# huzjkevin/planar_optical_flow

Hardware: AMD Instinct MI355X
Metric: scans/sec, flow-only preprocess of 450-pt synthetic scan pairs, batch 4096 per GPU (+ flow EPE vs reference oracle) (higher is better)
Workload: dtype f32 flow arithmetic (float32 outputs) + f64 exact association / mask decisions; the float64-output instantiation (the reference's float64 operation order) is `value_f64`

## Files before the change

### planar_optical_flow_amd/csrc/scan_flow.hip

```cpp
#include <cmath>
#include <type_traits>

#include "pof_common.h"

namespace {

constexpr int kThreads = 256;
constexpr int kFlatThreads = 128;
constexpr int kFlatRuns = 1;
constexpr int kFlatPairs = 64 * kFlatRuns;

__global__ void laser_phi_kernel(double start, double stop, double step, int n, double *tab)
{
    int i = blockIdx.x * blockDim.x + threadIdx.x;
    if (i >= n) return;
    double p = (double)i * step;
    p = p + start;
    if (i == n - 1 && n > 1) p = stop;
    double s, c;
    sincos(p, &s, &c);
    tab[i] = p;
    tab[n + 2 * i] = c;
    tab[n + 2 * i + 1] = s;
}
// ... 269 lines not shown
    if (a->det_offsets && slot >= cnt) {
        reinterpret_cast<float4 *>(img + kImgScreen)[slot] = make_float4(0.0f, 0.0f, INFINITY, 0.0f);
        img[40 + slot] = 0;
    }
}

__global__ __launch_bounds__(256) void scan_params_kernel(PreArgs a)
{
    params_work<true, true>(&a, blockIdx.x * blockDim.x + threadIdx.x);
}

__device__ __forceinline__ double to_sgpr(double v)
{
    const int lo = __builtin_amdgcn_readfirstlane(__double2loint(v));
    const int hi = __builtin_amdgcn_readfirstlane(__double2hiint(v));
    return __hiloint2double(hi, lo);
}

#define GLOBAL_AS __attribute__((address_space(1)))
using F4V = float __attribute__((ext_vector_type(4)));
using F2V = float __attribute__((ext_vector_type(2)));
using LL2V = long long __attribute__((ext_vector_type(2)));
__device__ __forceinline__ void stream_f4(float *base, long long idx4, float x, float y, float z, float w)
{
    F4V v = {x, y, z, w};
    __builtin_nontemporal_store(v, (GLOBAL_AS F4V *)base + idx4);
}
__device__ __forceinline__ void stream_f2(float *base, long long idx2, float x, float y)
{
    F2V v = {x, y};
    __builtin_nontemporal_store(v, (GLOBAL_AS F2V *)base + idx2);
}
__device__ __forceinline__ void stream_ll2(long long *base, long long idx2, long long x, long long y)
{
    LL2V v = {x, y};
    __builtin_nontemporal_store(v, (GLOBAL_AS LL2V *)base + idx2);
}

template <typename OutT>
__device__ __forceinline__ void store2(OutT *base, long long idx, double a, double b)
{
    using V = OutT __attribute__((ext_vector_type(2)));
    V v = {(OutT)a, (OutT)b};
    ((GLOBAL_AS V *)base)[idx] = v;
}

constexpr int kDetTile = 32;

__device__ __forceinline__ float4 prefilter_entry(double cx, double cy, double sd, double sa)
{
    const bool far = !(fabs(cx) + fabs(cy) < 100.0);
    return make_float4((float)cx, (float)cy, (float)sd, far ? INFINITY : (float)sa);
}

template <typename OutT, int PTS, int SPB>
__device__ __forceinline__ void scan_main(const PreArgs &a, const int block_y)
{
    __shared__ double s_det[SPB][kDetTile][5];
    __shared__ int s_lab[SPB][kDetTile];
    __shared__ float4 s_detf[SPB][kDetTile];

    const int b0 = block_y * SPB;
    const int tid = threadIdx.x;
    const int i0 = (blockIdx.x * kThreads + tid) * PTS;
    const int N = a.N;
    const bool live = i0 < N;
    const bool want_flow = a.flow != nullptr;
    const bool want_assoc = a.det_offsets != nullptr;

    int ndet[SPB];
    float r[SPB][PTS];
    double mot[SPB][7];
#pragma unroll
    for (int q = 0; q < SPB; ++q) {
        const int b = min(b0 + q, a.B - 1);
        const float *row = a.ranges + (long long)b * a.sample_stride;
#pragma unroll
        for (int k = 0; k < PTS; ++k) r[q][k] = 0.0f;
        if (live) {
            if (PTS == 2) {
                float2 v = *reinterpret_cast<const float2 *>(row + i0);
                r[q][0] = v.x;
                r[q][PTS - 1] = v.y;
            } else {
                r[q][0] = row[i0];
            }
        }
#pragma unroll
        for (int c = 0; c < 7; ++c) mot[q][c] = 0.0;
        ndet[q] = 0;
        if (want_flow || want_assoc) {
            typedef const __attribute__((address_space(4))) double *cptr;
            cptr m = (cptr)(a.ws_rec + (long long)b * kRecStride);
#pragma unroll
            for (int c = 0; c < 7; ++c) mot[q][c] = m[c];
            ndet[q] = (int)m[7];
        }
    }
    double cs[PTS], sn[PTS];
#pragma unroll
    for (int k = 0; k < PTS; ++k) cs[k] = sn[k] = 0.0;
    if (live) {
#pragma unroll
        for (int k = 0; k < PTS; ++k) {
            double2 t = *reinterpret_cast<const double2 *>(a.tab + N + 2 * (i0 + k));
            cs[k] = t.x;
            sn[k] = t.y;
        }
    }
    if (want_assoc) {
        const int qsel = tid / kInline, j = tid - qsel * kInline;
#pragma unroll
        for (int q = 0; q < SPB; ++q) {
            if (qsel == q) {
                const int b = min(b0 + q, a.B - 1);
                const double *w = a.ws_rec + (long long)b * kRecStride + 8 + j * kDetStride;
                s_det[q][j][0] = w[0];
                s_det[q][j][1] = w[1];
                s_det[q][j][2] = w[2];
                s_det[q][j][3] = w[3];
                s_det[q][j][4] = w[5];
                s_lab[q][j] = (int)w[4];
                s_detf[q][j] = prefilter_entry(w[0], w[1], w[3], w[5]);
            }
        }
    }
    bool synced = false;

#pragma unroll
    for (int q = 0; q < SPB; ++q) {
        const int b = b0 + q;
        const bool ok = live && b < a.B;
        double px[PTS], py[PTS];
#pragma unroll
        for (int k = 0; k < PTS; ++k) {
            px[k] = (double)r[q][k] * cs[k];
            py[k] = (double)r[q][k] * sn[k];
        }
        float pxf[PTS], pyf[PTS];
        bool far[PTS];
#pragma unroll
        for (int k = 0; k < PTS; ++k) {
            pxf[k] = (float)px[k];
            pyf[k] = (float)py[k];
            far[k] = !(fabsf(pxf[k]) + fabsf(pyf[k]) < 100.0f);
        }
        const long long o = (long long)b * N + i0;

        if (ok && a.xy) {
            OutT *xy = static_cast<OutT *>(a.xy);
#pragma unroll
            for (int k = 0; k < PTS; ++k) store2<OutT>(xy, o + k, px[k], py[k]);
        }

        if (ok && want_flow) {
            OutT *fl = static_cast<OutT *>(a.flow);
            const double m0 = mot[q][0], m1 = mot[q][1], m2 = mot[q][2], m3 = mot[q][3];
            const double t0 = mot[q][4], t1 = mot[q][5], dph = mot[q][6];
            double fxs[PTS], fys[PTS];
#pragma unroll
            for (int k = 0; k < PTS; ++k) {
                double fx, fy;
                apply_motion(a.flow_kind, px[k], py[k], m0, m1, m2, m3, t0, t1, dph, fx, fy);
                if (a.canonical) {
                    double gx = cs[k] * fx + (-sn[k]) * fy;
                    double gy = sn[k] * fx + cs[k] * fy;
                    fx = gx;
                    fy = gy;
                }
                fxs[k] = fx;
                fys[k] = fy;
            }
            if (PTS == 2 && sizeof(OutT) == 4) {
                stream_f4(reinterpret_cast<float *>(fl), o / 2, (float)fxs[0], (float)fys[0], (float)fxs[PTS - 1],
                          (float)fys[PTS - 1]);
            } else {
#pragma unroll
                for (int k = 0; k < PTS; ++k) store2<OutT>(fl, o + k, fxs[k], fys[k]);
            }
        }

        float vmask[PTS], dmask[PTS];
#pragma unroll
        for (int k = 0; k < PTS; ++k) {
            vmask[k] = (r[q][k] >= 20.0f) ? 0.0f : 1.0f;
            dmask[k] = 1.0f;
        }

        if (want_assoc) {
            double best[PTS];
            int bidx[PTS];
#pragma unroll
            for (int k = 0; k < PTS; ++k) {
                best[k] = 0.0;
                bidx[k] = 0;
            }
            if (!synced) {
                __syncthreads();
                synced = true;
            }
            int dfirst = 0;
            if (ndet[q] > kInline) dfirst = a.det_offsets[min(b, a.B - 1)];
            for (int base = 0; base < ndet[q]; base += (base == 0 ? kInline : kDetTile)) {
                const int cnt = min(base == 0 ? kInline : kDetTile, ndet[q] - base);
                if (base != 0) {
                    __syncthreads();
                    if (tid < cnt) {
                        const double *w = a.ws_det + (long long)(dfirst + base + tid) * kDetStride;
                        s_det[q][tid][0] = w[0];
                        s_det[q][tid][1] = w[1];
                        s_det[q][tid][2] = w[2];
                        s_det[q][tid][3] = w[3];
                        s_det[q][tid][4] = w[5];
                        s_lab[q][tid] = (int)w[4];
                        s_detf[q][tid] = prefilter_entry(w[0], w[1], w[3], w[5]);
                    }
                    __syncthreads();
                }
                float4 fnext = s_detf[q][0];
                for (int j = 0; j < cnt; ++j) {
                    const float4 f = fnext;
                    fnext = s_detf[q][min(j + 1, kDetTile - 1)];
                    bool exact[PTS];
                    bool any_exact = false;
#pragma unroll
                    for (int k = 0; k < PTS; ++k) {
                        const float exf = pxf[k] - f.x, eyf = pyf[k] - f.y;
                        const float s2f = fmaf(exf, exf, eyf * eyf);
                        const float mgn = fmaf(s2f, 1e-4f, 1e-3f);
                        exact[k] = far[k] || (s2f - mgn < f.w) || (fabsf(s2f - f.z) <= mgn);
                        if (!exact[k] && s2f < f.z) dmask[k] = 0.0f;
                        any_exact |= exact[k];
                    }
                    if (any_exact) {
                        const double cx = s_det[q][j][0], cy = s_det[q][j][1];
                        const double sd = s_det[q][j][3], sa = s_det[q][j][4];
#pragma unroll
                        for (int k = 0; k < PTS; ++k) {
                            if (!exact[k]) continue;
                            const double ex = px[k] - cx, ey = py[k] - cy;
                            const double s2 = ex * ex + ey * ey;
                            if (s2 <= sd) dmask[k] = 0.0f;
                            if (s2 <= sa) {
                                const double v = sqrt(s2) - s_det[q][j][2];
                                if (v < best[k]) {
                                    best[k] = v;
                                    bidx[k] = base + j + 1;
                                }
                            }
                        }
                    }
                }
            }
            if (ok) {
                long long cls[PTS];
                float gx[PTS], gy[PTS];
#pragma unroll
                for (int k = 0; k < PTS; ++k) {
                    cls[k] = 0;
                    gx[k] = gy[k] = 0.0f;
                    if (bidx[k] > 0) {
                        double wx, wy;
                        if (ndet[q] <= kInline) {
                            wx = s_det[q][bidx[k] - 1][0];
                            wy = s_det[q][bidx[k] - 1][1];
                            cls[k] = s_lab[q][bidx[k] - 1];
                        } else {
                            const double *w = a.ws_det + (long long)(dfirst + bidx[k] - 1) * kDetStride;
                            wx = w[0];
                            wy = w[1];
                            cls[k] = (long long)w[4];
                        }
                        gx[k] = (float)(wy * cs[k] - wx * sn[k]);
                        gy[k] = (float)((wx * cs[k] + wy * sn[k]) - (double)r[q][k]);
                    }
                }
                if (PTS == 2) {
                    if (a.closest) stream_ll2(reinterpret_cast<long long *>(a.closest), o / 2, bidx[0], bidx[PTS - 1]);
                    if (a.target_cls) stream_ll2(reinterpret_cast<long long *>(a.target_cls), o / 2, cls[0], cls[PTS - 1]);
                    if (a.target_reg) stream_f4(a.target_reg, o / 2, gx[0], gy[0], gx[PTS - 1], gy[PTS - 1]);
                } else {
                    if (a.closest) a.closest[o] = bidx[0];
                    if (a.target_cls) a.target_cls[o] = cls[0];
                    if (a.target_reg) reinterpret_cast<float2 *>(a.target_reg)[o] = make_float2(gx[0], gy[0]);
                }
            }
        }

        if (ok) {
            if (PTS == 2) {
                if (a.dyn_mask) stream_f2(a.dyn_mask, o / 2, dmask[0], dmask[PTS - 1]);
                if (a.valid_mask) stream_f2(a.valid_mask, o / 2, vmask[0], vmask[PTS - 1]);
                if (a.exclude_mask) stream_f2(a.exclude_mask, o / 2, dmask[0] * vmask[0], dmask[PTS - 1] * vmask[PTS - 1]);
            } else {
                if (a.dyn_mask) a.dyn_mask[o] = dmask[0];
                if (a.valid_mask) a.valid_mask[o] = vmask[0];
                if (a.exclude_mask) a.exclude_mask[o] = dmask[0] * vmask[0];
            }
        }
    }
}

constexpr int kMaxSlots = POF_SCAN_MAX_SLOTS;
constexpr int kWaveLds = 2 * kImgBytes;

enum : unsigned {
    kOutXy = 1u << 0, kOutFlow = 1u << 1, kHasDets = 1u << 2, kOutClosest = 1u << 3, kOutCls = 1u << 4,
    kOutReg = 1u << 5, kOutDyn = 1u << 6, kOutValid = 1u << 7, kOutExcl = 1u << 8, kCanonical = 1u << 9,
    kKindShift = 10,
};
constexpr int kCfgHeadline = (int)(kOutFlow | kHasDets | kOutCls | kOutReg | kOutExcl | kCanonical);

struct FlatBatch {
    const float *ranges;
    long long sample_stride;
    void *xy, *flow;
    int64_t *closest, *target_cls;
    float *target_reg, *dyn_mask, *valid_mask, *exclude_mask;
    const int32_t *det_offsets;
    const double *ws_rec, *ws_det;
    int B;
    int wave0;
};
static_assert(sizeof(FlatBatch) % 8 == 0, "FlatBatch is read from the kernel arguments in 8-byte words");

struct FlatArgs {
    const double *tab;
    const float *tabf;
    int N, halfN;
    unsigned magic_m;
    int magic_s;
    unsigned flags;
    int nb;
    int total_waves;
    int main_blocks;
    double ra[3], sd[3], sa[3];
    int lb[3];
    float m_dyn;
    float thr_assoc;
    float m_assoc;
    int uni_waves;
    unsigned uni_m;
    int uni_s;
    int pad_[2];
    int wave0[kMaxSlots];
    FlatBatch b[kMaxSlots];
};

struct ParamsMulti {
    int nb;
    int first, total;
    int uni_blocks;
    unsigned uni_m;
    int uni_s;
    int blk0[kMaxSlots + 1];
    PreArgs p[kMaxSlots];
};

template <typename T>
__device__ __forceinline__ T fma_t(T a, T b, T c);
template <>
__device__ __forceinline__ double fma_t<double>(double a, double b, double c) { return fma(a, b, c); }
template <>
__device__ __forceinline__ float fma_t<float>(float a, float b, float c) { return fmaf(a, b, c); }

template <typename T>
__device__ __forceinline__ void apply_motion_t(int kind, T px, T py, T m0, T m1, T m2, T m3, T t0, T t1, T dph,
                                               T &fx, T &fy)
{
    if (kind == 0) {
        fx = fma_t<T>(py, m1, px * m0) - t0;
        fy = fma_t<T>(py, m3, px * m2) - t1;
    } else if (kind == 1) {
        fx = (fma_t<T>(py, m1, px * m0) - t0) - px;
        fy = (fma_t<T>(py, m3, px * m2) - t1) - py;
    } else if (kind == 2) {
        fx = -t0 - (py * -dph);
        fy = -t1 - (px * dph);
    } else if (kind == 3) {
        fx = ((T)0 - m0 * py + m1) * m3;
        fy = ((m0 * px - (T)0) + m2) * m3;
    } else {
        fx = fma_t<T>(py, m1, px * m0) + t0;
        fy = fma_t<T>(py, m3, px * m2) + t1;
    }
}

template <int CFG>
struct FlatCfg {
    unsigned rt;
    __device__ __forceinline__ bool has(unsigned bit) const { return CFG >= 0 ? ((unsigned)CFG & bit) != 0 : (rt & bit) != 0; }
    __device__ __forceinline__ int kind() const { return CFG >= 0 ? (CFG >> kKindShift) & 7 : (int)(rt >> kKindShift) & 7; }
};

using D2V = double __attribute__((ext_vector_type(2)));

struct RunLoads {
    float2 rv;
    float4 tf;
    D2V t0v, t1v;
    int local, q;
    bool ok;
};

template <typename OutT>
__device__ __forceinline__ RunLoads flat_loads(const FlatArgs &L, const FlatBatch &bt, const int lane, const int sA,
                                               const int l0)
{
    constexpr bool kF32 = sizeof(OutT) == 4;
    RunLoads in;
    int local = l0 + lane;
    const int q = local >= L.halfN ? 1 : 0;
    local -= q ? L.halfN : 0;
    in.local = local;
    in.q = q;
    in.ok = sA + q < bt.B;
    const unsigned i0 = 2u * (unsigned)local;
    const GLOBAL_AS float *rowA = (const GLOBAL_AS float *)bt.ranges + (long long)sA * bt.sample_stride;
    const unsigned roff = (q && in.ok ? (unsigned)bt.sample_stride : 0u) + i0;
    const F2V rr = *(const GLOBAL_AS F2V *)(rowA + roff);
    in.rv = make_float2(rr.x, rr.y);
    in.tf = make_float4(0.f, 0.f, 0.f, 0.f);
    in.t0v = D2V{0.0, 0.0};
    in.t1v = D2V{0.0, 0.0};
    if (kF32 && L.tabf) {
        in.tf = *reinterpret_cast<const float4 *>(L.tabf + 2u * i0);
    } else {
        const double *tab_cs = L.tab + L.N;
        in.t0v = *reinterpret_cast<const D2V *>(tab_cs + 2u * i0);
        in.t1v = *reinterpret_cast<const D2V *>(tab_cs + 2u * i0 + 2);
    }
    return in;
}

template <typename OutT, int CFG>
__device__ __forceinline__ void flat_run(const FlatArgs &L, const FlatBatch &bt, const FlatCfg<CFG> cfg,
                                         const unsigned char *lds, const int lane, const int sA, const int l0,
                                         const long long pair0, const RunLoads &in)
{
    constexpr bool kF32 = sizeof(OutT) == 4;
    const int halfN = L.halfN, N = L.N;
    const int local = in.local, q = in.q;
    const int b = sA + q;
    const bool ok = in.ok;
    const int i0 = 2 * local;
    const float2 rv = in.rv;
    const double *tab_cs = L.tab + N;
    float csf[2], snf[2];
    const D2V t0v = in.t0v, t1v = in.t1v;
    if (kF32 && L.tabf) {
        csf[0] = in.tf.x; snf[0] = in.tf.y; csf[1] = in.tf.z; snf[1] = in.tf.w;
    } else {
        csf[0] = (float)t0v.x; snf[0] = (float)t0v.y; csf[1] = (float)t1v.x; snf[1] = (float)t1v.y;
    }
    const float r[2] = {rv.x, rv.y};
    F2V pxf = {r[0] * csf[0], r[1] * csf[1]}, pyf = {r[0] * snf[0], r[1] * snf[1]};
    auto cs64 = [&](int k) { return tab_cs[2u * (unsigned)(i0 + k)]; };
    auto sn64 = [&](int k) { return tab_cs[2u * (unsigned)(i0 + k) + 1]; };
    auto p64x = [&](int k) { return (double)r[k] * cs64(k); };
    auto p64y = [&](int k) { return (double)r[k] * sn64(k); };
    const unsigned char *hdr = lds + q * kImgBytes;

    if (cfg.has(kOutXy) && ok) {
        OutT *xy = static_cast<OutT *>(bt.xy) + 4 * pair0;
        store2<OutT>(xy, 2u * (unsigned)lane, p64x(0), p64y(0));
        store2<OutT>(xy, 2u * (unsigned)lane + 1, p64x(1), p64y(1));
    }

    if (cfg.has(kOutFlow)) {
        const int kind = cfg.kind();
        if (kF32 && kind != 1) {
            const float4 ma = *reinterpret_cast<const float4 *>(hdr);
            const float4 mb = *reinterpret_cast<const float4 *>(hdr + 16);
            float fxs[2], fys[2];
#pragma unroll
            for (int k = 0; k < 2; ++k) {
                float fx, fy;
                apply_motion_t<float>(kind, pxf[k], pyf[k], ma.x, ma.y, ma.z, ma.w, mb.x, mb.y, mb.z, fx, fy);
                if (cfg.has(kCanonical)) {
                    const float gx = fmaf(csf[k], fx, -snf[k] * fy);
                    const float gy = fmaf(snf[k], fx, csf[k] * fy);
                    fx = gx;
                    fy = gy;
                }
                fxs[k] = fx;
                fys[k] = fy;
            }
            if (ok) stream_f4(reinterpret_cast<float *>(bt.flow) + 4 * pair0, (unsigned)lane, fxs[0], fys[0], fxs[1], fys[1]);
        } else {
            const double *mot = reinterpret_cast<const double *>(hdr + kImgMot);
            const double m0 = mot[0], m1 = mot[1], m2 = mot[2], m3 = mot[3];
            const double tr0 = mot[4], tr1 = mot[5], dph = mot[6];
            OutT *fl = static_cast<OutT *>(bt.flow) + 4 * pair0;
            double cs[2], sn[2];
            if (kF32 && L.tabf) {
                cs[0] = cs64(0); sn[0] = sn64(0); cs[1] = cs64(1); sn[1] = sn64(1);
            } else {
                cs[0] = t0v.x; sn[0] = t0v.y; cs[1] = t1v.x; sn[1] = t1v.y;
            }
            double f[4];
#pragma unroll
            for (int k = 0; k < 2; ++k) {
                double fx, fy;
                apply_motion(kind, (double)r[k] * cs[k], (double)r[k] * sn[k], m0, m1, m2, m3, tr0, tr1, dph, fx, fy);
                if (cfg.has(kCanonical)) {
                    const double gx = cs[k] * fx + (-sn[k]) * fy;
                    const double gy = sn[k] * fx + cs[k] * fy;
                    fx = gx;
                    fy = gy;
                }
                f[2 * k] = fx;
                f[2 * k + 1] = fy;
            }
            if (ok) {
                if (kF32) {
                    stream_f4(reinterpret_cast<float *>(fl), (unsigned)lane, (float)f[0], (float)f[1], (float)f[2], (float)f[3]);
                } else {
                    D2V v0 = {f[0], f[1]}, v1 = {f[2], f[3]};
                    GLOBAL_AS D2V *dst = (GLOBAL_AS D2V *)fl + 2u * (unsigned)lane;
                    __builtin_nontemporal_store(v0, dst);
                    __builtin_nontemporal_store(v1, dst + 1);
                }
            }
        }
    }

    float vmask[2], dmask[2];
#pragma unroll
    for (int k = 0; k < 2; ++k) {
        vmask[k] = (r[k] >= 20.0f) ? 0.0f : 1.0f;
        dmask[k] = 1.0f;
    }

    if (cfg.has(kHasDets)) {
        const bool want_assoc = cfg.has(kOutClosest) || cfg.has(kOutCls) || cfg.has(kOutReg);
        const bool want_dyn = cfg.has(kOutDyn) || cfg.has(kOutExcl);
        const int4 h1 = *reinterpret_cast<const int4 *>(hdr + 16);
        const int2 h2 = *reinterpret_cast<const int2 *>(hdr + 32);
        const int2 h3 = *reinterpret_cast<const int2 *>(hdr + 40);
        const int nd = ok ? h1.w : 0;
        const int n_in = min(nd, kInline);
        const int nA = l0 < halfN ? reinterpret_cast<const int *>(lds)[7] : 0;
        const int nB = l0 + 63 >= halfN ? reinterpret_cast<const int *>(lds + kImgBytes)[7] : 0;
        const int n_loop = __builtin_amdgcn_readfirstlane(min(max(nA, nB), kInline));
        F2V mind = {INFINITY, INFINITY};
        const unsigned char *ent = hdr + kImgScreen;
        for (int j = 0; j < n_loop; ++j) {
            const float4 e = *reinterpret_cast<const float4 *>(ent + 16 * j);
            const F2V cx2 = {e.x, e.x}, cy2 = {e.y, e.y}, ns2 = {e.z, e.z};
            const F2V ex = pxf - cx2, ey = pyf - cy2;
            F2V d = __builtin_elementwise_fma(ey, ey, ns2);
            d = __builtin_elementwise_fma(ex, ex, d);
            mind = __builtin_elementwise_min(mind, d);
        }
        const bool samp_far = (h3.x | h3.y) != 0;
        int bidx[2] = {0, 0};
        int dfirst = 0;
        auto cls_of = [&](int j) { return ((j < 4 ? h2.x : h2.y) >> (8 * (j & 3))) & 3; };
        auto sel3 = [&](const double *v, int c) { return c == 0 ? v[0] : (c == 1 ? v[1] : v[2]); };
        auto candidate = [&](int k, int j1, double s2, double ra) {
            if (bidx[k] != 0) {
                double wx, wy, wra;
                if (bidx[k] <= kInline) {
                    const D2V c = *reinterpret_cast<const D2V *>(hdr + kImgCtr + 16 * (bidx[k] - 1));
                    wx = c.x; wy = c.y; wra = sel3(L.ra, cls_of(bidx[k] - 1));
                } else {
                    const GLOBAL_AS double *w = (const GLOBAL_AS double *)bt.ws_det + (long long)(dfirst + bidx[k] - 1) * kDetStride;
                    wx = w[0]; wy = w[1]; wra = w[2];
                }
                const double exd = p64x(k) - wx, eyd = p64y(k) - wy;
                if (!(sqrt(s2) - ra < sqrt(exd * exd + eyd * eyd) - wra)) return;
            }
            bidx[k] = j1;
        };
#pragma unroll
        for (int k = 0; k < 2; ++k) {
            const bool exk = samp_far || !(fabsf(pxf[k]) + fabsf(pyf[k]) < 100.0f);
            bool need_dyn = false;
            if (!exk && mind[k] <= -L.m_dyn) dmask[k] = 0.0f;
            else need_dyn = want_dyn && (exk || mind[k] <= L.m_dyn);
            bool need_assoc = want_assoc && (exk || mind[k] <= L.thr_assoc);
            if (need_assoc && !exk) {
                int ncand = 0, jc = 0;
                bool unsure = false;
                for (int j = 0; j < n_in; ++j) {
                    const float4 e = *reinterpret_cast<const float4 *>(ent + 16 * j);
                    const float exf = pxf[k] - e.x, eyf = pyf[k] - e.y;
                    const float d = fmaf(exf, exf, fmaf(eyf, eyf, e.z));
                    if (d <= e.w + L.m_assoc) {
                        if (d <= e.w - L.m_assoc) { ++ncand; jc = j; }
                        else unsure = true;
                    }
                }
                if (!unsure && ncand <= 1) {
                    if (ncand == 1) bidx[k] = jc + 1;
                    need_assoc = false;
                }
            }
            if (need_dyn || need_assoc) {
                const double pxd = p64x(k), pyd = p64y(k);
                for (int j = 0; j < n_in; ++j) {
                    const D2V c = *reinterpret_cast<const D2V *>(hdr + kImgCtr + 16 * j);
                    const int cl = cls_of(j);
                    const double exd = pxd - c.x, eyd = pyd - c.y;
                    const double s2 = exd * exd + eyd * eyd;
                    if (need_dyn && s2 <= sel3(L.sd, cl)) dmask[k] = 0.0f;
                    if (need_assoc && s2 <= sel3(L.sa, cl)) candidate(k, j + 1, s2, sel3(L.ra, cl));
                }
            }
        }
        if (nd > kInline) {
            dfirst = ((const GLOBAL_AS int32_t *)bt.det_offsets)[b];
            for (int j = kInline; j < nd; ++j) {
                const GLOBAL_AS double *w = (const GLOBAL_AS double *)bt.ws_det + (long long)(dfirst + j) * kDetStride;
                const double cx = w[0], cy = w[1], ra = w[2], sd = w[3], sa = w[5];
#pragma unroll
                for (int k = 0; k < 2; ++k) {
                    const double exd = p64x(k) - cx, eyd = p64y(k) - cy;
                    const double s2 = exd * exd + eyd * eyd;
                    if (s2 <= sd) dmask[k] = 0.0f;
                    if (want_assoc && s2 <= sa) candidate(k, j + 1, s2, ra);
                }
            }
        }
        if (ok && want_assoc) {
            long long cls[2];
            float gx[2], gy[2];
#pragma unroll
            for (int k = 0; k < 2; ++k) {
                cls[k] = 0;
                gx[k] = gy[k] = 0.0f;
                if (bidx[k] > 0) {
                    double wx, wy;
                    if (bidx[k] <= kInline) {
                        const D2V c = *reinterpret_cast<const D2V *>(hdr + kImgCtr + 16 * (bidx[k] - 1));
                        wx = c.x; wy = c.y;
                        const int cl = cls_of(bidx[k] - 1);
                        cls[k] = cl == 0 ? L.lb[0] : (cl == 1 ? L.lb[1] : L.lb[2]);
                    } else {
                        const GLOBAL_AS double *w = (const GLOBAL_AS double *)bt.ws_det + (long long)(dfirst + bidx[k] - 1) * kDetStride;
                        wx = w[0];
                        wy = w[1];
                        cls[k] = (long long)w[4];
                    }
                    const double c = cs64(k), sn_ = sn64(k);
                    gx[k] = (float)(wy * c - wx * sn_);
                    gy[k] = (float)((wx * c + wy * sn_) - (double)r[k]);
                }
            }
            if (cfg.has(kOutClosest)) stream_ll2(reinterpret_cast<long long *>(bt.closest) + 2 * pair0, (unsigned)lane, bidx[0], bidx[1]);
            if (cfg.has(kOutCls)) stream_ll2(reinterpret_cast<long long *>(bt.target_cls) + 2 * pair0, (unsigned)lane, cls[0], cls[1]);
            if (cfg.has(kOutReg)) stream_f4(bt.target_reg + 4 * pair0, (unsigned)lane, gx[0], gy[0], gx[1], gy[1]);
        }
    }

    if (ok) {
        if (cfg.has(kOutDyn)) stream_f2(bt.dyn_mask + 2 * pair0, (unsigned)lane, dmask[0], dmask[1]);
        if (cfg.has(kOutValid)) stream_f2(bt.valid_mask + 2 * pair0, (unsigned)lane, vmask[0], vmask[1]);
        if (cfg.has(kOutExcl)) stream_f2(bt.exclude_mask + 2 * pair0, (unsigned)lane, dmask[0] * vmask[0], dmask[1] * vmask[1]);
    }
}

typedef const __attribute__((address_space(4))) unsigned char *kernarg_ptr;
template <typename S>
__device__ __forceinline__ S kernarg_struct(kernarg_ptr p)
{
    static_assert(sizeof(S) % 8 == 0, "kernarg slots are read in 8-byte words");
    S out;
    unsigned long long *w = reinterpret_cast<unsigned long long *>(&out);
#pragma unroll
    for (int i = 0; i < (int)(sizeof(S) / 8); ++i)
        w[i] = *reinterpret_cast<const __attribute__((address_space(4))) unsigned long long *>(p + 8 * i);
    return out;
}
constexpr size_t kFlatArgsKernargBytes = (sizeof(FlatArgs) + 7) & ~(size_t)7;

template <typename OutT, int CFG>
__global__ __launch_bounds__(kFlatThreads, 8) void scan_flat_kernel(const FlatArgs L, const ParamsMulti P)
{
    constexpr int WAVES = kFlatThreads / 64;
    __shared__ __align__(16) unsigned char smem[WAVES][kWaveLds];
    kernarg_ptr ka = (kernarg_ptr)__builtin_amdgcn_kernarg_segment_ptr();
    int sblock = (int)blockIdx.x;
    if (sblock >= P.first) {
        if (sblock < P.first + P.total) {
            const int blk = sblock - P.first;
            int k = 0, b0 = P.blk0[0];
            if (P.uni_blocks) {
                k = (int)(__umulhi((unsigned)blk, P.uni_m) >> P.uni_s);
                b0 = k * P.uni_blocks;
            } else {
#pragma unroll
                for (int i = 1; i < kMaxSlots; ++i) k += (blk >= P.blk0[i]) ? 1 : 0;
                k = __builtin_amdgcn_readfirstlane(k);
#pragma unroll
                for (int i = 1; i < kMaxSlots; ++i) b0 = (k >= i) ? P.blk0[i] : b0;
            }
            const auto *pa = reinterpret_cast<const __attribute__((address_space(4))) PreArgs *>(
                ka + kFlatArgsKernargBytes + offsetof(ParamsMulti, p) + (size_t)k * sizeof(PreArgs));
            params_work<false, false>(pa, (blk - b0) * kFlatThreads + (int)threadIdx.x);
            return;
        }
        sblock -= P.total;
    }
    const int wv = __builtin_amdgcn_readfirstlane((int)threadIdx.x >> 6);
    const int lane = (int)threadIdx.x & 63;
    const int w = sblock * WAVES + wv;
    if (w >= L.total_waves) return;
    int k = 0;
    if (L.uni_waves) {
        k = (int)(__umulhi((unsigned)w, L.uni_m) >> L.uni_s);
    } else {
#pragma unroll
        for (int i = 1; i < kMaxSlots; ++i) k += (w >= L.wave0[i]) ? 1 : 0;
    }
    k = __builtin_amdgcn_readfirstlane(k);
    const FlatBatch bt = kernarg_struct<FlatBatch>(ka + offsetof(FlatArgs, b) + (size_t)k * sizeof(FlatBatch));
    const FlatCfg<CFG> cfg{L.flags};
    unsigned char *lds = smem[wv];

    const unsigned p0 = (unsigned)(w - bt.wave0) * (unsigned)kFlatPairs;
    const int sA = (int)(__umulhi(p0, L.magic_m) >> L.magic_s);
    const int l0 = (int)(p0 - (unsigned)sA * (unsigned)L.halfN);

    RunLoads in[kFlatRuns];
#pragma unroll
    for (int c = 0; c < kFlatRuns; ++c) in[c] = flat_loads<OutT>(L, bt, lane, sA, l0 + 64 * c);

    if (cfg.has(kOutFlow) || cfg.has(kHasDets)) {
        {
            const int sq = lane >> 5, i = lane & 31;
            if (i < kImgBytes / 16) {
                const double *rec = bt.ws_rec + (long long)min(sA + sq, bt.B - 1) * kRecStride;
                *reinterpret_cast<F4V *>(lds + sq * kImgBytes + 16 * i) = ((const GLOBAL_AS F4V *)(rec + kRecImg))[i];
            }
        }
        __builtin_amdgcn_fence(__ATOMIC_RELEASE, "wavefront");
        __builtin_amdgcn_wave_barrier();
        __builtin_amdgcn_fence(__ATOMIC_ACQUIRE, "wavefront");
    }
#pragma unroll
    for (int c = 0; c < kFlatRuns; ++c)
        flat_run<OutT, CFG>(L, bt, cfg, lds, lane, sA, l0 + 64 * c, (long long)p0 + 64 * c, in[c]);
}

template <typename T>
__global__ void rotate_flow_kernel(const T *in, T *out, const double *tab, long long total, int N,
                                   int to_canonical)
{
    long long p = (long long)blockIdx.x * blockDim.x + threadIdx.x;
    if (p >= total) return;
    int i = (int)(p % N);
    T gx, gy;
    pof_rotate_flow_point<T>(tab[N + 2 * i], tab[N + 2 * i + 1], in[2 * p], in[2 * p + 1], to_canonical, gx, gy);
    out[2 * p] = gx;
    out[2 * p + 1] = gy;
}

__global__ void det_to_canonical_kernel(const float *ranges, const double *tab, const double *det_r,
                                        const double *det_phi, double *dx, double *dy, long long total,
                                        int N)
{
    long long p = (long long)blockIdx.x * blockDim.x + threadIdx.x;
    if (p >= total) return;
    int i = (int)(p % N);
    double s, c;
    sincos(det_phi[p] - tab[i], &s, &c);
    dx[p] = s * det_r[p];
    dy[p] = c * det_r[p] - (double)ranges[p];
}

__global__ void canonical_to_det_kernel(const float *ranges, const double *tab, const double *dx,
                                        const double *dy, double *det_r, double *det_phi,
                                        long long total, int N)
{
    long long p = (long long)blockIdx.x * blockDim.x + threadIdx.x;
    if (p >= total) return;
    int i = (int)(p % N);
    double ty = (double)ranges[p] + dy[p];
    double tphi = atan2(dx[p], ty);
    det_phi[p] = tphi + tab[i];
    det_r[p] = ty / cos(tphi);
}

template <typename OutT, int PTS, int SPB>
__global__ __launch_bounds__(kThreads, 8) void scan_preprocess_kernel(PreArgs a)
{
    scan_main<OutT, PTS, SPB>(a, blockIdx.y);
}

template <typename OutT, int PTS, int SPB>
__global__ __launch_bounds__(kThreads, 8) void scan_preprocess_chain_kernel(PreArgs a, PreArgs nx, int main_rows)
{
    if ((int)blockIdx.y >= main_rows) {
        if (blockIdx.x == 0) params_work<false, true>(&nx, ((int)blockIdx.y - main_rows) * kThreads + threadIdx.x);
        return;
    }
    scan_main<OutT, PTS, SPB>(a, blockIdx.y);
}

__global__ __launch_bounds__(256) void flow_from_xy_kernel(const double *xy, const double *odom0,
                                                           const double *odom1, int kind, int canonical,
                                                           const double *tab, double *out, int N)
{
    __shared__ double s_sc[4];
    __shared__ double s_mot[8];
    const int b = blockIdx.x;
    const double *o0 = odom0 + 3 * b, *o1 = odom1 + 3 * b;
    if (threadIdx.x < 2) {
        const int which = threadIdx.x;
        const double ang = motion_angle(kind, which, o0, o1);
        sincos(ang, &s_sc[2 * which], &s_sc[2 * which + 1]);
    }
    __syncthreads();
    if (threadIdx.x == 0) motion_params(kind, o0, o1, s_sc[0], s_sc[1], s_sc[2], s_sc[3], s_mot);
    __syncthreads();
    for (int i = threadIdx.x; i < N; i += blockDim.x) {
        const long long p = (long long)b * N + i;
        const double px = xy[2 * p], py = xy[2 * p + 1];
        double fx, fy;
        apply_motion(kind, px, py, s_mot[0], s_mot[1], s_mot[2], s_mot[3], s_mot[4], s_mot[5], s_mot[6], fx, fy);
        if (canonical) {
            const double c = tab[N + 2 * i], sn = tab[N + 2 * i + 1];
            const double gx = c * fx + (-sn) * fy, gy = sn * fx + c * fy;
            fx = gx;
            fy = gy;
        }
        out[2 * p] = fx;
        out[2 * p + 1] = fy;
    }
}

__global__ void xy_to_rphi_kernel(const double *x, const double *y, double *r, double *phi, long long n)
{
    long long p = (long long)blockIdx.x * blockDim.x + threadIdx.x;
    if (p >= n) return;
    r[p] = hypot(x[p], y[p]);
    phi[p] = atan2(y[p], x[p]);
}

}

extern "C" int pof_flow_from_xy(const double *xy, const double *odom0, const double *odom1, int flow_kind,
                                int canonical, const double *tab, double *flow, int B, int N,
                                pof_stream_t stream)
{
    POF_CLEAR_STALE_ERROR();
    if (!xy || !odom0 || !odom1 || !flow || B < 0 || N < 1) return POF_E_BADARG;
    if (flow_kind < 0 || flow_kind > 4) return POF_E_BADARG;
    if (canonical && !tab) return POF_E_BADARG;
    if (B == 0) return POF_OK;
    flow_from_xy_kernel<<<B, 256, 0, pof_stream(stream)>>>(xy, odom0, odom1, flow_kind, canonical, tab, flow, N);
    POF_CHECK_LAUNCH();
    return POF_OK;
}

extern "C" int pof_xy_to_rphi(const double *x, const double *y, double *r, double *phi, long long n,
                              pof_stream_t stream)
{
    POF_CLEAR_STALE_ERROR();
    if (!x || !y || !r || !phi || n < 0) return POF_E_BADARG;
    if (n == 0) return POF_OK;
    xy_to_rphi_kernel<<<(unsigned)((n + 255) / 256), 256, 0, pof_stream(stream)>>>(x, y, r, phi, n);
    POF_CHECK_LAUNCH();
    return POF_OK;
}

extern "C" int pof_laser_phi(double angle_inc, int num_pts, double *tab, pof_stream_t stream)
{
    POF_CLEAR_STALE_ERROR();
    if (!tab || num_pts < 2) return POF_E_BADARG;
    const double fov = (double)(num_pts - 1) * angle_inc;
    const double start = -fov * 0.5, stop = fov * 0.5;
    const double step = (stop - start) / (double)(num_pts - 1);
    laser_phi_kernel<<<(num_pts + 255) / 256, 256, 0, pof_stream(stream)>>>(start, stop, step, num_pts, tab);
    POF_CHECK_LAUNCH();
    return POF_OK;
}

static double sq_threshold(double r, bool strict)
{
    if (!(r > 0.0)) return (!strict && r == 0.0) ? 0.0 : -1.0;
    auto ok = [&](double s) { double q = std::sqrt(s); return strict ? (q < r) : (q <= r); };
    double c = r * r;
    for (int it = 0; it < 64 && !ok(c); ++it) c = std::nextafter(c, 0.0);
    for (int it = 0; it < 64; ++it) {
        double up = std::nextafter(c, HUGE_VAL);
        if (!ok(up)) break;
        c = up;
    }
    return c;
}

extern "C" size_t pof_scan_preprocess_workspace_bytes(int B, int D)
{
    if (B < 0 || D < 0) return 0;
    return ((size_t)B * kRecStride + (size_t)D * kDetStride) * sizeof(double) + 64;
}

namespace {

void fill_class_constants(PreArgs &a, bool have_dets, const double *assoc_radius, const int32_t *labels,
                          const double *dyn_radius)
{
    double thr[6] = {0, 0, 0, 0, 0, 0};
    if (have_dets)
        for (int k = 0; k < 3; ++k) {
            thr[k] = sq_threshold(dyn_radius[k], false);
            thr[3 + k] = sq_threshold(assoc_radius[k], true);
        }
    a.ra0 = have_dets ? assoc_radius[0] : 0.0; a.ra1 = have_dets ? assoc_radius[1] : 0.0;
    a.ra2 = have_dets ? assoc_radius[2] : 0.0;
    a.sd0 = thr[0]; a.sd1 = thr[1]; a.sd2 = thr[2];
    a.sa0 = thr[3]; a.sa1 = thr[4]; a.sa2 = thr[5];
    a.lb0 = have_dets ? labels[0] : 0; a.lb1 = have_dets ? labels[1] : 0; a.lb2 = have_dets ? labels[2] : 0;
}

void bind_workspace(PreArgs &a, void *workspace, int B)
{
    uintptr_t base = (reinterpret_cast<uintptr_t>(workspace) + 63) & ~(uintptr_t)63;
    a.ws_rec = reinterpret_cast<double *>(base);
    a.ws_det = a.ws_rec + (size_t)B * kRecStride;
}

float f32_round_up(double v)
{
    float f = (float)v;
    if ((double)f < v) f = std::nextafter(f, INFINITY);
    return f;
}

struct FlatCommon {
    const double *tab;
    const float *tabf;
    int N, flow_kind, canonical, out_f64;
    const double *assoc_radius, *dyn_radius;
    const int32_t *labels;
};

bool flat_shape_ok(int N) { return N % 2 == 0 && N >= 2 * kFlatPairs; }

unsigned flat_flags(const FlatBatch &b, const FlatCommon &c)
{
    unsigned f = 0;
    if (b.xy) f |= kOutXy;
    if (b.flow) f |= kOutFlow;
    if (b.det_offsets) f |= kHasDets;
    if (b.closest) f |= kOutClosest;
    if (b.target_cls) f |= kOutCls;
    if (b.target_reg) f |= kOutReg;
    if (b.dyn_mask) f |= kOutDyn;
    if (b.valid_mask) f |= kOutValid;
    if (b.exclude_mask) f |= kOutExcl;
    if (c.canonical) f |= kCanonical;
    f |= (unsigned)c.flow_kind << kKindShift;
    return f;
}

int bind_next(const pof_scan_inputs *next, PreArgs &nx, int *jobs)
{
    *jobs = 0;
    if (next->B < 0 || next->D < 0 || next->B > 65535) return POF_E_BADARG;
    if (next->want_flow && (!next->odom0 || !next->odom1)) return POF_E_BADARG;
    if (next->flow_kind < 0 || next->flow_kind > 4) return POF_E_BADARG;
    if (next->det_offsets && next->D > 0 && (!next->det_rphi || !next->det_cls)) return POF_E_BADARG;
    if (next->B > 0 && (next->want_flow || next->det_offsets)) {
        if (!next->workspace ||
            next->workspace_bytes < pof_scan_preprocess_workspace_bytes(next->B, next->det_offsets ? next->D : 0))
            return POF_E_WORKSPACE;
        nx.B = next->B; nx.D = next->det_offsets ? next->D : 0;
        nx.odom0 = next->odom0; nx.odom1 = next->odom1; nx.flow_kind = next->flow_kind;
        nx.flow = next->want_flow ? reinterpret_cast<void *>(1) : nullptr;
        nx.det_offsets = next->det_offsets; nx.det_rphi = next->det_rphi; nx.det_cls = next->det_cls;
        fill_class_constants(nx, next->det_offsets != nullptr, next->assoc_radius, next->labels, next->dyn_radius);
        bind_workspace(nx, next->workspace, next->B);
        *jobs = params_job_count(nx.B);
    }
    return POF_OK;
}

void magic_u31(unsigned d, unsigned *m, int *sh)
{
    int lg = 1;
    while ((1u << lg) < d) ++lg;
    *m = (unsigned)(((1ull << (31 + lg)) + d - 1) / d);
    *sh = lg - 1;
}

int launch_flat(const FlatBatch *cur, int n_cur, const FlatCommon &c, const pof_scan_inputs *const *next, int n_next,
                hipStream_t s)
{
    FlatArgs L = {};
    L.tab = c.tab; L.tabf = c.tabf; L.N = c.N; L.halfN = c.N / 2;
    int lg = 0;
    while ((1u << lg) < (unsigned)L.halfN) ++lg;
    L.magic_m = (unsigned)(((1ull << (31 + lg)) + (unsigned)L.halfN - 1) / (unsigned)L.halfN);
    L.magic_s = lg - 1;
    L.flags = flat_flags(cur[0], c);
    L.nb = n_cur;
    PreArgs cc = {};
    fill_class_constants(cc, cur[0].det_offsets != nullptr, c.assoc_radius, c.labels, c.dyn_radius);
    L.ra[0] = cc.ra0; L.ra[1] = cc.ra1; L.ra[2] = cc.ra2;
    L.sd[0] = cc.sd0; L.sd[1] = cc.sd1; L.sd[2] = cc.sd2;
    L.sa[0] = cc.sa0; L.sa[1] = cc.sa1; L.sa[2] = cc.sa2;
    L.lb[0] = cc.lb0; L.lb[1] = cc.lb1; L.lb[2] = cc.lb2;
    double md = 0.0, ma = 0.0, gap = -HUGE_VAL, span = 0.0;
    for (int k = 0; k < 3; ++k) {
        md = std::fmax(md, 1e-3 + 1e-4 * std::fmax(L.sd[k], 0.0));
        ma = std::fmax(ma, 1e-3 + 1e-4 * std::fmax(std::fmax(L.sd[k], L.sa[k]), 0.0));
        gap = std::fmax(gap, L.sa[k] - L.sd[k]);
        span = std::fmax(span, std::fabs(L.sa[k] - L.sd[k]));
    }
    L.m_dyn = f32_round_up(md * (1.0 + 1e-6));
    L.m_assoc = f32_round_up(ma * 1.001 + 2.4e-7 * span);
    L.thr_assoc = f32_round_up(gap + (double)L.m_assoc + 1e-6 * std::fabs(gap));
    long long waves = 0;
    const long long pairs_per_wave = kFlatPairs;
    for (int i = 0; i < n_cur; ++i) {
        if (flat_flags(cur[i], c) != L.flags) return POF_E_BADARG;
        L.b[i] = cur[i];
        L.b[i].wave0 = (int)waves;
        L.wave0[i] = (int)waves;
        waves += ((long long)cur[i].B * L.halfN + pairs_per_wave - 1) / pairs_per_wave;
        if ((long long)cur[i].B * L.halfN >= (1LL << 31) || waves >= (1LL << 30)) return POF_E_SHAPE;
    }
    for (int i = n_cur; i < kMaxSlots; ++i) L.wave0[i] = 0x7fffffff;
    L.total_waves = (int)waves;
    L.uni_waves = 0; L.uni_m = 0; L.uni_s = 0;
    if (n_cur > 0 && waves % n_cur == 0) {
        const long long per = waves / n_cur;
        bool same = per > 1;
        for (int i = 0; i < n_cur && same; ++i) same = L.wave0[i] == (int)(per * i);
        if (same) { L.uni_waves = (int)per; magic_u31((unsigned)per, &L.uni_m, &L.uni_s); }
    }
    const int wpb = kFlatThreads / 64;
    L.main_blocks = (int)((waves + wpb - 1) / wpb);
    ParamsMulti P = {};
    P.nb = 0;
    int extra = 0;
    for (int i = 0; i < n_next; ++i) {
        PreArgs nx = {};
        int jobs = 0;
        const int rc = bind_next(next[i], nx, &jobs);
        if (rc != POF_OK) return rc;
        if (jobs == 0) continue;
        P.blk0[P.nb] = extra;
// ... 292 lines not shown
```

Baseline: 399.5 million.

## Stash f64 trig table in LDS, drop f32 table, fuse two-point association walk

Always loads the f64 cos/sin pairs and derives the f32 values from them, removing the separate f32 table load. The f64 values are written to a per-wave LDS stash so later uses read LDS instead of re-fetching global memory. The candidate-detection walk now handles both points of a lane in one loop, sharing each entry load. The second sample's header is only copied when the run crosses a sample boundary. In exchange, LDS per wave grows, which may reduce occupancy, and the f64 table loads are now wider on the default f32 path.

```diff
diff --git a/planar_optical_flow_amd/csrc/scan_flow.hip b/planar_optical_flow_amd/csrc/scan_flow.hip
--- a/planar_optical_flow_amd/csrc/scan_flow.hip
+++ b/planar_optical_flow_amd/csrc/scan_flow.hip
@@ -595,7 +595,9 @@
 }
 
 constexpr int kMaxSlots = POF_SCAN_MAX_SLOTS;
-constexpr int kWaveLds = 2 * kImgBytes;
+constexpr int kStashOff = 2 * kImgBytes;
+constexpr int kStashBytes = 64 * 32;
+constexpr int kWaveLds = kStashOff + kFlatRuns * kStashBytes;
 
 enum : unsigned {
     kOutXy = 1u << 0, kOutFlow = 1u << 1, kHasDets = 1u << 2, kOutClosest = 1u << 3, kOutCls = 1u << 4,
@@ -690,7 +692,6 @@
 
 struct RunLoads {
     float2 rv;
-    float4 tf;
     D2V t0v, t1v;
     int local, q;
     bool ok;
@@ -700,7 +701,6 @@
 __device__ __forceinline__ RunLoads flat_loads(const FlatArgs &L, const FlatBatch &bt, const int lane, const int sA,
                                                const int l0)
 {
-    constexpr bool kF32 = sizeof(OutT) == 4;
     RunLoads in;
     int local = l0 + lane;
     const int q = local >= L.halfN ? 1 : 0;
@@ -713,43 +713,30 @@
     const unsigned roff = (q && in.ok ? (unsigned)bt.sample_stride : 0u) + i0;
     const F2V rr = *(const GLOBAL_AS F2V *)(rowA + roff);
     in.rv = make_float2(rr.x, rr.y);
-    in.tf = make_float4(0.f, 0.f, 0.f, 0.f);
-    in.t0v = D2V{0.0, 0.0};
-    in.t1v = D2V{0.0, 0.0};
-    if (kF32 && L.tabf) {
-        in.tf = *reinterpret_cast<const float4 *>(L.tabf + 2u * i0);
-    } else {
-        const double *tab_cs = L.tab + L.N;
-        in.t0v = *reinterpret_cast<const D2V *>(tab_cs + 2u * i0);
-        in.t1v = *reinterpret_cast<const D2V *>(tab_cs + 2u * i0 + 2);
-    }
+    const double *tab_cs = L.tab + L.N;
+    in.t0v = *reinterpret_cast<const D2V *>(tab_cs + 2u * i0);
+    in.t1v = *reinterpret_cast<const D2V *>(tab_cs + 2u * i0 + 2);
     return in;
 }
 
 template <typename OutT, int CFG>
 __device__ __forceinline__ void flat_run(const FlatArgs &L, const FlatBatch &bt, const FlatCfg<CFG> cfg,
-                                         const unsigned char *lds, const int lane, const int sA, const int l0,
-                                         const long long pair0, const RunLoads &in)
+                                         const unsigned char *lds, const unsigned char *stash, const int lane,
+                                         const int sA, const int l0, const long long pair0, const RunLoads &in)
 {
     constexpr bool kF32 = sizeof(OutT) == 4;
-    const int halfN = L.halfN, N = L.N;
-    const int local = in.local, q = in.q;
+    const int halfN = L.halfN;
+    const int q = in.q;
     const int b = sA + q;
     const bool ok = in.ok;
-    const int i0 = 2 * local;
     const float2 rv = in.rv;
-    const double *tab_cs = L.tab + N;
-    float csf[2], snf[2];
     const D2V t0v = in.t0v, t1v = in.t1v;
-    if (kF32 && L.tabf) {
-        csf[0] = in.tf.x; snf[0] = in.tf.y; csf[1] = in.tf.z; snf[1] = in.tf.w;
-    } else {
-        csf[0] = (float)t0v.x; snf[0] = (float)t0v.y; csf[1] = (float)t1v.x; snf[1] = (float)t1v.y;
-    }
+    const float csf[2] = {(float)t0v.x, (float)t1v.x}, snf[2] = {(float)t0v.y, (float)t1v.y};
     const float r[2] = {rv.x, rv.y};
     F2V pxf = {r[0] * csf[0], r[1] * csf[1]}, pyf = {r[0] * snf[0], r[1] * snf[1]};
-    auto cs64 = [&](int k) { return tab_cs[2u * (unsigned)(i0 + k)]; };
-    auto sn64 = [&](int k) { return tab_cs[2u * (unsigned)(i0 + k) + 1]; };
+    const double *st64 = reinterpret_cast<const double *>(stash) + 4 * lane;
+    auto cs64 = [&](int k) { return st64[2 * k]; };
+    auto sn64 = [&](int k) { return st64[2 * k + 1]; };
     auto p64x = [&](int k) { return (double)r[k] * cs64(k); };
     auto p64y = [&](int k) { return (double)r[k] * sn64(k); };
     const unsigned char *hdr = lds + q * kImgBytes;
@@ -785,12 +772,7 @@
             const double m0 = mot[0], m1 = mot[1], m2 = mot[2], m3 = mot[3];
             const double tr0 = mot[4], tr1 = mot[5], dph = mot[6];
             OutT *fl = static_cast<OutT *>(bt.flow) + 4 * pair0;
-            double cs[2], sn[2];
-            if (kF32 && L.tabf) {
-                cs[0] = cs64(0); sn[0] = sn64(0); cs[1] = cs64(1); sn[1] = sn64(1);
-            } else {
-                cs[0] = t0v.x; sn[0] = t0v.y; cs[1] = t1v.x; sn[1] = t1v.y;
-            }
+            const double cs[2] = {t0v.x, t1v.x}, sn[2] = {t0v.y, t1v.y};
             double f[4];
 #pragma unroll
             for (int k = 0; k < 2; ++k) {
@@ -866,30 +848,41 @@
             }
             bidx[k] = j1;
         };
+        bool need_dyn_[2], need_assoc_[2], walk[2];
 #pragma unroll
         for (int k = 0; k < 2; ++k) {
             const bool exk = samp_far || !(fabsf(pxf[k]) + fabsf(pyf[k]) < 100.0f);
-            bool need_dyn = false;
+            need_dyn_[k] = false;
             if (!exk && mind[k] <= -L.m_dyn) dmask[k] = 0.0f;
-            else need_dyn = want_dyn && (exk || mind[k] <= L.m_dyn);
-            bool need_assoc = want_assoc && (exk || mind[k] <= L.thr_assoc);
-            if (need_assoc && !exk) {
-                int ncand = 0, jc = 0;
-                bool unsure = false;
-                for (int j = 0; j < n_in; ++j) {
-                    const float4 e = *reinterpret_cast<const float4 *>(ent + 16 * j);
+            else need_dyn_[k] = want_dyn && (exk || mind[k] <= L.m_dyn);
+            need_assoc_[k] = want_assoc && (exk || mind[k] <= L.thr_assoc);
+            walk[k] = need_assoc_[k] && !exk;
+        }
+        if (walk[0] || walk[1]) {
+            int ncand[2] = {0, 0}, jc[2] = {0, 0};
+            bool unsure[2] = {false, false};
+            for (int j = 0; j < n_in; ++j) {
+                const float4 e = *reinterpret_cast<const float4 *>(ent + 16 * j);
+#pragma unroll
+                for (int k = 0; k < 2; ++k) {
                     const float exf = pxf[k] - e.x, eyf = pyf[k] - e.y;
                     const float d = fmaf(exf, exf, fmaf(eyf, eyf, e.z));
-                    if (d <= e.w + L.m_assoc) {
-                        if (d <= e.w - L.m_assoc) { ++ncand; jc = j; }
-                        else unsure = true;
+                    if (walk[k] && d <= e.w + L.m_assoc) {
+                        if (d <= e.w - L.m_assoc) { ++ncand[k]; jc[k] = j; }
+                        else unsure[k] = true;
                     }
                 }
-                if (!unsure && ncand <= 1) {
-                    if (ncand == 1) bidx[k] = jc + 1;
-                    need_assoc = false;
+            }
+#pragma unroll
+            for (int k = 0; k < 2; ++k)
+                if (walk[k] && !unsure[k] && ncand[k] <= 1) {
+                    if (ncand[k] == 1) bidx[k] = jc[k] + 1;
+                    need_assoc_[k] = false;
                 }
-            }
+        }
+#pragma unroll
+        for (int k = 0; k < 2; ++k) {
+            const bool need_dyn = need_dyn_[k], need_assoc = need_assoc_[k];
             if (need_dyn || need_assoc) {
                 const double pxd = p64x(k), pyd = p64y(k);
                 for (int j = 0; j < n_in; ++j) {
@@ -919,6 +912,12 @@
         if (ok && want_assoc) {
             long long cls[2];
             float gx[2], gy[2];
+            D2V wcs[2] = {D2V{0.0, 0.0}, D2V{0.0, 0.0}};
+            if (bidx[0] > 0 || bidx[1] > 0) {
+                const D2V *tp = reinterpret_cast<const D2V *>(stash) + 2 * lane;
+                wcs[0] = tp[0];
+                wcs[1] = tp[1];
+            }
 #pragma unroll
             for (int k = 0; k < 2; ++k) {
                 cls[k] = 0;
@@ -936,7 +935,7 @@
                         wy = w[1];
                         cls[k] = (long long)w[4];
                     }
-                    const double c = cs64(k), sn_ = sn64(k);
+                    const double c = wcs[k].x, sn_ = wcs[k].y;
                     gx[k] = (float)(wy * c - wx * sn_);
                     gy[k] = (float)((wx * c + wy * sn_) - (double)r[k]);
                 }
@@ -1023,18 +1022,26 @@
     if (cfg.has(kOutFlow) || cfg.has(kHasDets)) {
         {
             const int sq = lane >> 5, i = lane & 31;
-            if (i < kImgBytes / 16) {
+            const bool spans = l0 + 64 * kFlatRuns - 1 >= L.halfN;
+            if (i < kImgBytes / 16 && (sq == 0 || spans)) {
                 const double *rec = bt.ws_rec + (long long)min(sA + sq, bt.B - 1) * kRecStride;
                 *reinterpret_cast<F4V *>(lds + sq * kImgBytes + 16 * i) = ((const GLOBAL_AS F4V *)(rec + kRecImg))[i];
             }
         }
-        __builtin_amdgcn_fence(__ATOMIC_RELEASE, "wavefront");
-        __builtin_amdgcn_wave_barrier();
-        __builtin_amdgcn_fence(__ATOMIC_ACQUIRE, "wavefront");
-    }
+    }
+#pragma unroll
+    for (int c = 0; c < kFlatRuns; ++c) {
+        D2V *st = reinterpret_cast<D2V *>(lds + kStashOff + c * kStashBytes) + 2 * lane;
+        st[0] = in[c].t0v;
+        st[1] = in[c].t1v;
+    }
+    __builtin_amdgcn_fence(__ATOMIC_RELEASE, "wavefront");
+    __builtin_amdgcn_wave_barrier();
+    __builtin_amdgcn_fence(__ATOMIC_ACQUIRE, "wavefront");
 #pragma unroll
     for (int c = 0; c < kFlatRuns; ++c)
-        flat_run<OutT, CFG>(L, bt, cfg, lds, lane, sA, l0 + 64 * c, (long long)p0 + 64 * c, in[c]);
+        flat_run<OutT, CFG>(L, bt, cfg, lds, lds + kStashOff + c * kStashBytes, lane, sA, l0 + 64 * c,
+                            (long long)p0 + 64 * c, in[c]);
 }
 
 template <typename T>
```

Result: faster. 411.2 million, median of 4 (+2.9%).
